# AzheeeQAQ/Game-of-life-distributed

Hardware: AMD Instinct MI355X
Metric: cell-updates/sec (GCUPS) at 1/2/4/8 MI355X; % of HBM roofline (higher is better)
Workload: dtype u32 bit-sliced (1 bit/cell)

## Files before the change

game-of-life-distributed_amd/csrc/gol_kernels.h:

```cpp
#pragma once
#include <hip/hip_runtime.h>
#include <stdint.h>

#include "gol_limits.h"
#include "gol_pad_plan.h"

namespace golk {

constexpr int kHalo = 128;
constexpr int kWave = 64;
constexpr int kTileValid = 62;
constexpr int kHalfTileValid = 30;

struct RowMap {
    int base;
    int wrap;
    int off;
    int rmax;
};

struct StepArgs {
    const uint32_t *src;
    uint32_t *dst;
    int W;
// ... 9 lines not shown

hipError_t launch_step_tb(const StepArgs &a, int depth, hipStream_t s, bool fill_skip, int wpl, bool paired = false);
int max_depth_for(int wpl);
int persist_max_depth(int wpl);
int tb_tiles(int Ww, int wpl);
hipError_t launch_step_generic(const StepArgs &a, hipStream_t s);
int tb_waves(const StepArgs &a, int wpl);
int tb_blocks_per_cu(int depth, int wpl);
int tb_wave_slots_per_cu(int depth, int wpl, bool paired);
int auto_rows_per_wave(int Ww, int rows, int depth, int wave_slots, bool fill_skip, int wpl, bool paired = false);

struct SkewArgs {
    StepArgs base;
    int tiles_x;
    int tx;
    int half;
    int nst;
    int wgt[8];
    int hcap;
    int prio_young;
    unsigned *error;
    unsigned long long *trace;
    int pairs;
};
bool skew_supported(int depth, int wpl, bool half = false, bool pr = false);
int skew_blocks_per_cu(int depth, int wpl, bool half = false, bool pr = false);
hipError_t launch_skew(const SkewArgs &p, int depth, int wpl, hipStream_t s);

struct PersistArgs {
    StepArgs base;
    uint32_t *buf0, *buf1;
    int first;
    int J;
    int half_last;
    int S;
    int S_old, S_young;
    int paired;
    int wg_tx, wg_sy;
    int cols, wg_y;
    int tiles_x;
    int nw;
    unsigned *progress;
    unsigned *error;
    long long timeout_ticks;
    unsigned long long *trace;
    int fault;
// ... 168 lines not shown
```

game-of-life-distributed_amd/csrc/gol_kernels.hip:

```cpp
#include "gol_kernels.h"
#include "gol_bits.h"
#include "gol_layout.h"
#include "gol_flip_seam.h"

#include <algorithm>
#include <climits>
#include <type_traits>
#include <utility>

namespace golk {
#ifndef GOL_LOOP_PAD
#define GOL_LOOP_PAD 0
#endif
#ifndef GOL_FILL_PHASES
#define GOL_FILL_PHASES 4
#endif

template <typename F, int... I>
__device__ __forceinline__ void static_for_impl(F &&f, std::integer_sequence<int, I...>) {
    (f(std::integral_constant<int, I>()), ...);
}
template <int N, typename F>
__device__ __forceinline__ void static_for(F &&f) {
    static_for_impl(f, std::make_integer_sequence<int, N>());
}

// ... 573 lines not shown
        if constexpr (WPL <= 2) parity_fix<1>();
        if (s < A) {
            hook(s, ii0, x0);
            stage<D, 0, WPL>(s, x0, h0, h1, cc);
        }
        if (s >= 1 && s - 1 < A) {
            hook(s - 1, ii0 + 1, x1);
            stage<D, 1, WPL>(s - 1, x1, h0, h1, cc);
        }
        if (s >= 2 && s - 2 < A) {
            hook(s - 2, ii0 + 2, x2);
            stage<D, 2, WPL>(s - 2, x2, h0, h1, cc);
        }
    }
}
#ifndef GOL_SKEW_WAIT_TRACE
#define GOL_SKEW_WAIT_TRACE 0
#endif
#ifndef GOL_SKEW_STORE_CPOL
#define GOL_SKEW_STORE_CPOL 16
#endif
template <int D>
struct SkewPlan {
    static constexpr int STEP = D > 20 ? 6 : 3;
    static constexpr int NPH = (D - 1) / STEP;
    static constexpr int P(int j) { return (j + 1) * STEP; }
    static constexpr int NROWS(int j) { return 2 * ((j + 1 < NPH ? P(j + 1) : D) - P(j)); }
    static constexpr int BASE(int j) {
        int b = 0;
        for (int i = 0; i < j; ++i) b += NROWS(i);
        return b;
    }
    static constexpr int NEXP = BASE(NPH);
    static_assert(NPH >= 1 && STEP % 3 == 0, "skew depth >= 4");
};


template <int D, int WPL>
struct PairSt {
    uint32_t a0[D][WPL], a1[D][WPL];
    uint32_t b0[D][WPL], b1[D][WPL];
    uint32_t p0[D][WPL], p1[D][WPL], p2[D][WPL];
    uint32_t c[D][WPL];
};

struct Shifted {
    uint32_t w, e;
// ... 158 lines not shown
                pair_unsum(st.p0[t][k], st.p1[t][k], st.a0[t][k], st.a1[t][k], h0[1][t][k], h1[1][t][k]);
            }
        }
}

template <int D, int LO, int WPL>
__device__ __forceinline__ void push_group_hi(Lanes<WPL> &x0, Lanes<WPL> &x1, Lanes<WPL> &x2,
                                              uint32_t (&h0)[3][D][WPL], uint32_t (&h1)[3][D][WPL],
                                              uint32_t (&cc)[3][D][WPL]) {
    parity_fix<1>();
#pragma unroll
    for (int s = LO; s < D + 2; ++s) {
        parity_fix<2>();
        if (s < D) stage<D, 0, WPL>(s, x0, h0, h1, cc);
        if (s - 1 >= LO && s - 1 < D) stage<D, 1, WPL>(s - 1, x1, h0, h1, cc);
        if (s - 2 >= LO) stage<D, 2, WPL>(s - 2, x2, h0, h1, cc);
    }
}

template <int D, int WPL, bool HALF = false, bool PR = false>
__device__ __forceinline__ uint32_t stream_skew(const StepArgs &a, int ab, int eb, int tile, bool self,
                                                uint32_t *exp_mine, const uint32_t *exp_next, int *flag_mine,
                                                int *flag_next, unsigned *error, unsigned long long *phase_tr,
                                                int dr = 0) {
    using SP = SkewPlan<D>;
    constexpr int ROW = 64 * WPL;
    constexpr int TV = HALF ? kHalfTileValid : kTileValid;
    const int lane = threadIdx.x & 63;
    const int hl = HALF ? (lane & 31) : lane;
    const int rofs = (HALF && lane >= 32) ? dr : 0;
    const int Ww = a.Ww;
    const int S = eb - ab;
    const int t0 = tile * TV * WPL;
    int col = (t0 + WPL * (hl - 1)) % Ww;
    if (col < 0) col += Ww;
    const bool keep = hl >= 1 && hl <= TV && (t0 + WPL * (hl - 1)) < Ww;
    int r = ab + rofs + a.in.off;
    const int wrap = a.in.wrap > 0 ? a.in.wrap : INT_MAX;
    if (a.in.wrap > 0) {
        r %= a.in.wrap;
        if (r < 0) r += a.in.wrap;
    }
    const uint32_t *__restrict__ src = a.src + col;
    auto load_next = [&]() -> Lanes<WPL> {
        const Lanes<WPL> v = load_row<WPL>(src + (size_t)(a.in.base + min(r, a.in.rmax)) * Ww);
        r = (r + 1 == wrap) ? 0 : r + 1;
        return v;
    };
    const __amdgpu_buffer_rsrc_t brs = __builtin_amdgcn_make_buffer_rsrc(
        a.dst + (size_t)(a.dst_base + ab + D) * Ww, (short)0, (S + (HALF ? dr : 0)) * Ww * 4, 0x00020000);
    const int clo = a.count_lo - (ab + D + rofs), chi = a.count_hi - (ab + D + rofs);
    const int colw = col + rofs * Ww;
    uint32_t cnt = 0;
    auto emit = [&](const Lanes<WPL> &y, int oi) {
        const bool ok = keep && (unsigned)oi < (unsigned)S;
// ... 47 lines not shown
            if constexpr (GOL_SKEW_WAIT_TRACE) wt0 = __builtin_amdgcn_s_memrealtime();
            x0 = vmov(n0);
            x1 = vmov(n1);
            x2 = vmov(n2);
            if constexpr (GOL_SKEW_WAIT_TRACE) {
                asm volatile("s_waitcnt vmcnt(0)" ::: "memory");
                wfill += __builtin_amdgcn_s_memrealtime() - wt0;
                ++nfill;
            }
        }
    };
    static_for<SP::NPH>([&](auto j) { fill(std::integral_constant<int, SP::P(decltype(j)::value)>()); });
    fill(std::integral_constant<int, D>());
    if (phase_tr && lane == 0) phase_tr[0] = (unsigned long long)__builtin_amdgcn_s_memrealtime();
    asm volatile("s_waitcnt lgkmcnt(0)" ::: "memory");
    if (lane == 0) __hip_atomic_store(flag_mine, 1, __ATOMIC_RELAXED, __HIP_MEMORY_SCOPE_WORKGROUP);

    Lanes<WPL> q0, q1, q2;
#pragma unroll
    for (int i = 0; i < WPL; ++i) q0.w[i] = q1.w[i] = q2.w[i] = 0u;
    int qoi = -8;
    [[maybe_unused]] PairSt<D, WPL> st;
    [[maybe_unused]] Shifted sh = {0u, 0u};
    const int kmain = S + (self ? 2 * D : 2 * SP::P(0));
    for (int i = 0; i < GOL_LOOP_PAD; ++i) asm volatile("s_nop 0");
    if constexpr (PR) {
        constexpr int KSTART = 3 * ((2 * D + 2) / 3);
        static_assert(KSTART % 6 == 0, "the pair main loop starts at an even push");
        {
            pr_enter<D, 0, WPL>(h0, h1, cc, st);
            sh = row_shifts<WPL>(x0);
            for (; k < kmain; k += 6) {
                {
                    const Lanes<WPL> n0 = load_next(), n1 = load_next(), n2 = load_next();
                    emit(q0, qoi);
                    emit(q1, qoi + 1);
                    emit(q2, qoi + 2);
                    __builtin_amdgcn_sched_barrier(0);
                    Lanes<WPL> y0 = x0, y1 = x1, y2 = x2;
                    Lanes<WPL> xn;
                    push_group_pr<D, 0, WPL>(y0, y1, y2, st, sh, n0, xn);
                    q0 = y0;
                    q1 = y1;
                    q2 = y2;
                    qoi = k - 2 * D;
                    __builtin_amdgcn_sched_barrier(0);
                    x0 = xn;
                    if constexpr (HALF) x1 = vmov(n1); else x1 = vmov_even(n1);
                    x2 = vmov(n2);
                }
                {
                    const Lanes<WPL> n0 = load_next(), n1 = load_next(), n2 = load_next();
                    emit(q0, qoi);
                    emit(q1, qoi + 1);
                    emit(q2, qoi + 2);
                    __builtin_amdgcn_sched_barrier(0);
                    Lanes<WPL> y0 = x0, y1 = x1, y2 = x2;
                    Lanes<WPL> xn;
                    push_group_pr<D, 1, WPL>(y0, y1, y2, st, sh, n0, xn);
                    q0 = y0;
                    q1 = y1;
                    q2 = y2;
                    qoi = k + 3 - 2 * D;
                    __builtin_amdgcn_sched_barrier(0);
                    x0 = xn;
                    x1 = vmov(n1);
                    x2 = vmov(n2);
                }
            }
            if constexpr (D % 3 != 0) pr_leave<D, 0, WPL>(st, h0, h1, cc);
        }
    }
    for (; !PR && k < kmain; k += 3) {
        const Lanes<WPL> n0 = load_next(), n1 = load_next(), n2 = load_next();
        emit(q0, qoi);
        emit(q1, qoi + 1);
        emit(q2, qoi + 2);
        __builtin_amdgcn_sched_barrier(0);
        Lanes<WPL> y0 = x0, y1 = x1, y2 = x2;
        push_group<D, D, WPL>(y0, y1, y2, h0, h1, cc);
        q0 = y0;
        q1 = y1;
        q2 = y2;
        qoi = k - 2 * D;
        __builtin_amdgcn_sched_barrier(0);
        if constexpr (GOL_SKEW_WAIT_TRACE) wt0 = __builtin_amdgcn_s_memrealtime();
        x0 = vmov(n0);
        x1 = vmov(n1);
        x2 = vmov(n2);
        if constexpr (GOL_SKEW_WAIT_TRACE) {
            asm volatile("s_waitcnt vmcnt(3)" ::: "memory");
            wmain += __builtin_amdgcn_s_memrealtime() - wt0;
            ++nmain;
        }
    }
    if constexpr (GOL_SKEW_WAIT_TRACE) {
        if (phase_tr && lane == 0) {
            phase_tr[32] = wmain;
            phase_tr[33] = nmain;
            phase_tr[64] = wfill;
            phase_tr[65] = nfill;
        }
    }
    if (phase_tr && lane == 0) phase_tr[1] = (unsigned long long)__builtin_amdgcn_s_memrealtime();
    if (!self) {
        if (__hip_atomic_load(flag_next, __ATOMIC_RELAXED, __HIP_MEMORY_SCOPE_WORKGROUP) == 0) {
            const long long t_start = (long long)__builtin_amdgcn_s_memrealtime();
            while (__hip_atomic_load(flag_next, __ATOMIC_RELAXED, __HIP_MEMORY_SCOPE_WORKGROUP) == 0) {
                if ((long long)__builtin_amdgcn_s_memrealtime() - t_start > 200000000ll) {
                    if (error && lane == 0) __hip_atomic_store(error, 1u, __ATOMIC_RELAXED, __HIP_MEMORY_SCOPE_SYSTEM);
                    break;
                }
                __builtin_amdgcn_s_sleep(1);
            }
        }
        asm volatile("s_waitcnt lgkmcnt(0)" ::: "memory");
// ... 101 lines not shown
    const int tile = tc * p.tx + w % p.tx, pos = w / p.tx;
    if (lane == 0) s_flag[w] = 0;
    if (threadIdx.x == 0) s_cnt = 0;
    __syncthreads();
    if (tile >= p.tiles_x) return;
    if (p.prio_young && w >= 4) __builtin_amdgcn_s_setprio(1);
    const int L = HALF ? p.base.rows_out / 2 : p.base.rows_out;
    const int A0 = (int)((int64_t)stack * L / p.nst) - D, E0 = (int)((int64_t)(stack + 1) * L / p.nst) - D;
    const int64_t Ls = (int64_t)(E0 - A0) + p.hcap;
    int cum = 0, tot = 0;
    for (int q = 0; q < sy; ++q) {
        tot += p.wgt[q];
        cum += q < pos ? p.wgt[q] : 0;
    }
    const bool bottom = pos == sy - 1;
    constexpr int G = PR ? 6 : 3;
    const int ab = A0 + (int)(Ls * cum / tot) / G * G;
    const int eb = bottom ? E0 : A0 + (int)(Ls * (cum + p.wgt[pos]) / tot) / G * G;
    const long long t_start = p.trace ? (long long)__builtin_amdgcn_s_memrealtime() : 0;
    const uint32_t cnt = stream_skew<D, WPL, HALF, PR>(p.base, ab, eb, tile, bottom, s_exp[w], bottom ? nullptr : s_exp[w + p.tx],
                                             &s_flag[w], bottom ? nullptr : &s_flag[w + p.tx], p.error,
                                             (p.trace && blockIdx.x < 1024) ? p.trace + 8 + 2 * (blockIdx.x * 64 + 16 + w)
                                                                            : nullptr,
                                             L);
    if (p.trace && lane == 0 && blockIdx.x < 1024) {
        p.trace[8 + 2 * (blockIdx.x * 64 + w)] = (unsigned long long)t_start;
        p.trace[8 + 2 * (blockIdx.x * 64 + w) + 1] = (unsigned long long)__builtin_amdgcn_s_memrealtime();
    }
    if (p.base.alive) wg_count(p.base.alive, &s_cnt, cnt, sy * min(p.tx, p.tiles_x - tc * p.tx));
}

__host__ __device__ constexpr int persist_waves(int depth, int wpl) { return depth * wpl <= 16 ? 16 : 8; }

#ifndef GOL_PERSIST_WG_COUNT
#define GOL_PERSIST_WG_COUNT 1
#endif
template <int D, int WPL, int NW>
__global__ __launch_bounds__(NW * 64) void gol_persist_kernel(PersistArgs p) {
    const int lane = threadIdx.x & 63;
    const int w = __builtin_amdgcn_readfirstlane(threadIdx.x >> 6);
    const int b = blockIdx.x;
    const int wx = b % p.cols, wy = b / p.cols;
    const int tile = wx * p.wg_tx + w % p.wg_tx;
    int r0, band, dir = 1;
    const int ry = w / p.wg_tx;
    const bool paired = p.paired != 0;
    if (paired) {
// ... 1747 lines not shown
```

game-of-life-distributed_amd/csrc/golhip_impl.h:

```cpp
#pragma once
#include <hip/hip_runtime.h>
#include <rccl/rccl.h>

#include <algorithm>
#include <atomic>
#include <chrono>
#include <condition_variable>
#include <cstdint>
#include <cstring>
#include <memory>
#include <mutex>
#include <string>
#include <vector>

#include "../../include/golhip.h"
#include "gol_kernels.h"

#define GOLHIP_HIDDEN __attribute__((visibility("hidden")))

namespace gh GOLHIP_HIDDEN {

using golk::kHalo;

int fail(int code, const char *fmt, ...) __attribute__((format(printf, 2, 3)));
// ... 68 lines not shown
    bool own_stream = false;

    uint32_t *buf[2] = {nullptr, nullptr};
    int cur = 0;
    int64_t phys_rows = 0;

    int tb_depth = 20;
    int rows_per_wave = 0;
    int cu_count = 0;
    int dev_cu = 0;
    int fill_skip = 1;
    int last_variant = 1;
    int skew = 1;
    int skew_young = 0;
    int skew_hcap = -1;
    int skew_prio = 0;
    int skew_tx = 0;
    int skew_half = 0;
    int lds_bpc[4] = {};
    int64_t lds_bpc_bytes[4] = {};
    int lds_bpc_stride[4] = {};
    int skew_bpc[gh::kNumDepths][12] = {};
    int skew_pairs = 5;
    unsigned *skew_err = nullptr;
    unsigned *skew_err_dev = nullptr;
    int lds_band = -1;
    int lds_depth = 0;
    int lds_xcd = 1;
    int lds_waves = 0;
    int lds_wg_cu = 1;
    int lds_stride = 1;
    int resident_fault = 0;
    int lds_age = 0;
    int lds_pre = 2;
    gh::DevScratch<uint32_t> lds_edge;
    int persistent = -1;
    int wpl_opt = 0;
    bool no_quads = false;
    int persist_depth = 0;
    int persist_waves = 0;
    int paired_bands = 1;
    int dummy_rows = 0;
    int persist_wg_tx = 0;
    int persist_half = 1;
    unsigned long long *d_trace = nullptr;
    unsigned *d_sync = nullptr;
// ... 188 lines not shown
```

game-of-life-distributed_amd/csrc/golhip_options.cpp:

```cpp
#include "golhip_impl.h"
#include <climits>
#include <cstdio>
#include <cstdlib>
#include <initializer_list>
#include <string>

namespace gh GOLHIP_HIDDEN {

static bool measurement_env() {
    const char *v = getenv("GOLHIP_MEASUREMENT");
    return v && !strcmp(v, "1");
}
bool test_hooks_env() {
    const char *v = getenv("GOLHIP_TEST_HOOKS");
    return v && !strcmp(v, "1");
}
bool tuning_env() {
    const char *v = getenv("GOLHIP_TUNING");
    return (v && !strcmp(v, "1")) || measurement_env();
}

namespace {

enum Consent : unsigned { kProduct = 1, kTuning = 2, kMeasurement = 4, kTestHook = 8 };

constexpr int64_t kAny = INT64_MAX;

struct Option {
    const char *key;
    unsigned consent;
    int64_t lo, hi;
    uint32_t members;
    bool or_zero;
    int golhip::*field;
    bool boolean;
    bool clears_rpw;
    int (*handler)(golhip_t h, int64_t value);
};

int set_trace(golhip_t h, int64_t value) {
    if (value && !h->d_trace) {
        if (hipMalloc(&h->d_trace, kTraceWords * sizeof(unsigned long long)) != hipSuccess)
            return fail(GOLHIP_ENOMEM, "trace buffer");
        if (hipMemsetAsync(h->d_trace, 0, kTraceWords * sizeof(unsigned long long), h->stream) != hipSuccess ||
            hipStreamSynchronize(h->stream) != hipSuccess)
            return fail(GOLHIP_EHIP, "trace buffer memset");
    }
// ... 45 lines not shown
    {"persist_depth", kTuning, RANGE(0, GOLHIP_MAX_TB_DEPTH), &golhip::persist_depth, false, false, nullptr},
    {"persist_waves", kTuning, 0, 16, bits({0, 4, 8, 16}), false, &golhip::persist_waves, false, false, nullptr},
    {"dummy_rows", kTuning, RANGE(0, kHalo), &golhip::dummy_rows, false, false, nullptr},
    {"paired_bands", kTuning, RANGE(0, 1), &golhip::paired_bands, false, true, nullptr},
    {"persist_half", kTuning, RANGE(0, 1), &golhip::persist_half, false, false, nullptr},
    {"persist_wg_tx", kTuning, RANGE(0, 16), &golhip::persist_wg_tx, false, false, nullptr},
    {"trace", kTuning, BOOLEAN, nullptr, true, false, set_trace},
    {"cu_count", kTuning, BOOLEAN, nullptr, false, true, set_cu_count},
    {"fill_skip", kTuning, BOOLEAN, &golhip::fill_skip, true, true, nullptr},
    {"skew_young", kTuning, 10, 400, 0, true, &golhip::skew_young, false, false, nullptr},
    {"skew_hcap", kTuning, RANGE(-1, 256), &golhip::skew_hcap, false, false, nullptr},
    {"skew_prio", kTuning, RANGE(0, 1), &golhip::skew_prio, false, false, nullptr},
    {"skew_half", kTuning, RANGE(-1, 1), &golhip::skew_half, false, false, nullptr},
    {"skew_tx", kTuning, RANGE(0, 2), &golhip::skew_tx, false, false, nullptr},
    {"lds_depth", kTuning, RANGE(0, 64), &golhip::lds_depth, false, false, nullptr},
    {"lds_waves", kTuning, 0, 16, bits({0, 8, 16}), false, &golhip::lds_waves, false, false, nullptr},
    {"lds_wg_cu", kTuning, RANGE(1, 2), &golhip::lds_wg_cu, false, false, nullptr},
    {"lds_age", kTuning, 25, 400, 0, true, &golhip::lds_age, false, false, nullptr},
    {"lds_pre", kTuning, RANGE(0, 64), &golhip::lds_pre, false, false, nullptr},
    {"lds_stride", kTuning, RANGE(0, 1), &golhip::lds_stride, false, false, nullptr},
    {"lds_xcd", kTuning, RANGE(0, 1), &golhip::lds_xcd, false, false, nullptr},
    {"flip_overlap", kTuning, RANGE(0, 3), &golhip::flip_overlap, false, false, nullptr},
    {"skew_pairs", kTuning, RANGE(0, 7), &golhip::skew_pairs, false, false, nullptr},
    {"halo_skip", kMeasurement, BOOLEAN, &golhip::halo_skip, true, false, nullptr},
    {"resident_fault", kTestHook, RANGE(0, 2), &golhip::resident_fault, false, false, nullptr},
    {"resident_max_turns", kTestHook, RANGE(1, golk::kResidentMaxTurns), &golhip::resident_max, false, false, nullptr},
    {"flip_debug", kMeasurement | kTestHook, RANGE(0, 7), nullptr, false, false, set_flip_debug},
};
#undef RANGE
#undef BOOLEAN

const Option *find_option(const char *key) {
    for (const Option &o : kOptions)
        if (!strcmp(key, o.key)) return &o;
    return nullptr;
}

bool accepts(const Option &o, int64_t v) {
    if (o.or_zero && v == 0) return true;
    return v >= o.lo && v <= o.hi && (!o.members || (o.members >> v & 1));
}

int refuse(const Option &o, int64_t value) {
    if (!o.members)
        return fail(GOLHIP_EINVAL, "%s %lld not in %s%lld..%lld", o.key, (long long)value, o.or_zero ? "0 or " : "",
                    (long long)o.lo, (long long)o.hi);
// ... 33 lines not shown
    return info.c_str();
}

int golhip_set_tb_depth(golhip_t h, int32_t t) {
    if (int rc = check(h)) return rc;
    if (t < 1 || t > GOLHIP_MAX_TB_DEPTH) return fail(GOLHIP_EINVAL, "tb depth %d not in 1..%d", t, GOLHIP_MAX_TB_DEPTH);
    std::lock_guard<std::mutex> g(h->mu);
    h->tb_depth = t;
    return GOLHIP_OK;
}

int golhip_set_rows_per_wave(golhip_t h, int32_t r) {
    if (int rc = check(h)) return rc;
    if (r < 0) return fail(GOLHIP_EINVAL, "rows per wave %d", r);
    std::lock_guard<std::mutex> g(h->mu);
    h->rows_per_wave = r;
    return GOLHIP_OK;
}

int golhip_set_option(golhip_t h, const char *key, int64_t value) {
    if (int rc = check(h)) return rc;
    if (!key) return fail(GOLHIP_EINVAL, "null option");
    const Option *o = find_option(key);
    if (o && (o->consent & kTuning) && !tuning_env())
        return fail(GOLHIP_EINVAL, "%s is an A/B tuning knob of the kernel plans: set GOLHIP_TUNING=1", key);
    std::lock_guard<std::mutex> g(h->mu);
    if (!o) return fail(GOLHIP_EINVAL, "unknown option %s", key);
    if (!accepts(*o, value)) return refuse(*o, value);
    if (o->handler) {
        if (int rc = o->handler(h, value)) return rc;
    } else {
        if (value && (o->consent & kMeasurement) && !measurement_env())
            return fail(GOLHIP_EINVAL, "%s gives wrong results: measurement runs only (GOLHIP_MEASUREMENT=1)", key);
        if (value && (o->consent & kTestHook) && !test_hooks_env())
            return fail(GOLHIP_EINVAL, "%s is a test hook (GOLHIP_TEST_HOOKS=1)", key);
        h->*(o->field) = o->boolean ? value != 0 : (int)value;
    }
    if (o->clears_rpw)
        for (int &c : h->auto_rpw) c = 0;
    return GOLHIP_OK;
}

}
```

game-of-life-distributed_amd/csrc/golhip_pad.cpp:

```cpp
#include "golhip_impl.h"

namespace gh GOLHIP_HIDDEN {

bool pad_applies(golhip_t h) {
    golk::PadPlan p;
    return h->W % 32 != 0 && h->torus() && !h->ringed() && golk::pad_plan(h->W, &p);
}

struct PadRule {
    int64_t min_cells, min_turns;
};
static constexpr PadRule kPadRule[] = {
    {0, 2},
    {1000 * 1000, 1},
};
static bool pad_auto(int64_t cells, int64_t nturns) {
    for (const PadRule &r : kPadRule)
        if (cells >= r.min_cells && nturns >= r.min_turns) return true;
    return false;
}

bool pad_wanted(golhip_t h, int64_t nturns) {
    if (nturns < 1 || h->pad_mode == 0 || !pad_applies(h)) return false;
    if (h->pad_mode == 1) return true;
// ... 43 lines not shown
    return GOLHIP_OK;
}

static void take_settings(golhip_t h, golhip *w) {
    w->stream = h->stream;
    w->flags = h->flags;
    if (w->wpl_opt != h->wpl_opt || w->cu_count != h->cu_count || w->fill_skip != h->fill_skip ||
        w->paired_bands != h->paired_bands)
        for (int &c : w->auto_rpw) c = 0;
    w->wpl_opt = h->wpl_opt;
    w->cu_count = h->cu_count;
    w->fill_skip = h->fill_skip;
    w->paired_bands = h->paired_bands;
    w->tb_depth = h->tb_depth;
    w->rows_per_wave = h->rows_per_wave;
    w->dummy_rows = h->dummy_rows;
    w->skew = h->skew;
    w->skew_young = h->skew_young;
    w->skew_hcap = h->skew_hcap;
    w->skew_prio = h->skew_prio;
    w->skew_tx = h->skew_tx;
    w->skew_half = h->skew_half;
    w->skew_pairs = h->skew_pairs;
    w->d_trace = h->d_trace;
}

int pad_step(golhip_t h, int64_t nturns, bool *ran) {
    *ran = false;
    if (int rc = ensure_wide(h)) {
        if (h->pad_mode == 1 || rc != GOLHIP_ENOMEM) return rc;
        h->pad_nomem = true;
        return GOLHIP_OK;
    }
    golhip *w = h->wide;
    take_settings(h, w);
    w->il = want_il(w);
    w->loaded = true;
    golk::PadArgs a{};
    golk::pad_plan(h->W, &a.plan);
    a.canon = h->cur_rows();
    a.wide = w->cur_rows();
    a.rows = h->rows;
    a.Ww = h->Ww;
    a.Wwp = w->Ww;
    w->n = Counters{};
    HIP_OR_FAIL(golk::launch_pad(a, w->il, h->stream));
// ... 169 lines not shown
```

game-of-life-distributed_amd/csrc/golhip_plan.cpp:

```cpp
#include "golhip_impl.h"
#include <climits>
#include <functional>

namespace gh GOLHIP_HIDDEN {

int largest_depth(int64_t want) {
    for (int d : kDepths)
        if (d <= want && d != 9 && d != 18) return d;
    return 1;
}
static bool special_depth(int d) { return d == 9 || d == 18; }

DepthRun depth_plan(int cap, int64_t left) {
    const int M = special_depth(cap) ? cap : largest_depth(std::max(1, cap));
    if (left <= 0) return {M, 0};
    const int64_t head = std::max<int64_t>(0, left / M - 12);
    const int t = (int)(left - head * M);
    std::vector<int> nl(t + 1, INT_MAX), mn(t + 1, 0), pick(t + 1, 0);
    nl[0] = 0;
    mn[0] = INT_MAX;
    for (int v = 1; v <= t; ++v)
        for (int d : kDepths) {
            if (d > M || d > v || nl[v - d] == INT_MAX || (special_depth(d) && M != d)) continue;
            const int n = nl[v - d] + 1, m = std::min(mn[v - d], d);
// ... 158 lines not shown
                               : golk::tb_tiles(h->Ww, wpl);
        const int Lh = half ? L / 2 : L;
        for (int tx = 1; tx <= 2; ++tx) {
            if (h->skew_tx && tx != h->skew_tx) continue;
            const int sy = 8 / tx, tcols = (tiles + tx - 1) / tx;
            const int nst = std::min(h->cu_count * bpc / tcols,
                                     Lh / (sy * (smin + hcap) - hcap));
            if (nst < 1) continue;
            if (h->skew == 1 && (int64_t)nst * tcols * 4 < (int64_t)h->cu_count * bpc * 3) continue;
            if (((double)Lh / nst + hcap + (half ? Lh : 0)) * h->Ww * 4 >= 2147483648.0) continue;
            const double per_wave = ((double)Lh / nst + hcap) / sy * (half ? 1.02 : 1.0);
            if (per_wave < best * 0.999) {
                best = per_wave;
                best_tx = tx;
                best_nst = nst;
                best_half = half;
                best_tiles = tiles;
            }
        }
    }
    if (!best_tx) return false;
    sk->tiles_x = best_tiles;
    sk->pairs = pr ? 1 : 0;
    sk->tx = best_tx;
    sk->nst = best_nst;
    sk->half = best_half;
    sk->hcap = hcap;
    return true;
}

static bool skew_fills(golhip_t h) {
    if (!h->skew || h->W % 32 != 0) return false;
    const int wpl = wpl_per_launch(h);
    int cap = std::min(h->tb_depth, golk::max_depth_for(wpl));
    if (cap == 9 && wpl != 4) cap = 8;
    const int depth = cap == 9 ? 9 : largest_depth(cap);
    golk::SkewArgs sk{};
    return skew_dims(h, depth, wpl, sched_rows(h), &sk);
}

bool skew_plan(golhip_t h, int depth, int wpl, const golk::StepArgs &a, golk::SkewArgs *sk) {
    if (!skew_dims(h, depth, wpl, a.rows_out, sk)) return false;
    if (!h->skew_err) {
        void *p = nullptr, *d = nullptr;
        if (hipHostMalloc(&p, sizeof(unsigned), hipHostMallocMapped) != hipSuccess) return false;
        if (hipHostGetDevicePointer(&d, p, 0) != hipSuccess) {
// ... 80 lines not shown
        out->pre = h->lds_pre;
        const bool whole = wpl == 2 && P2 % 64 == 0;
        out->age = h->lds_age > 0 ? h->lds_age : !whole ? 100 : waves == 16 ? 60 : 70;
    }
    return true;
}

}

using namespace gh;

extern "C" {

int golhip_halo_schedule(int32_t strip_rows, int32_t tb_depth, int32_t resident, int64_t turns_left,
                         int32_t *depth, int32_t *launches) {
    if (!depth || !launches || strip_rows <= 0 || tb_depth < 1 || tb_depth > GOLHIP_MAX_TB_DEPTH || turns_left < 1)
        return fail(GOLHIP_EINVAL, "bad halo schedule request");
    const HaloRun hr = halo_next(std::min(tb_depth, strip_rows), strip_rows, resident != 0, turns_left);
    *depth = hr.d;
    *launches = hr.k;
    return GOLHIP_OK;
}

int golhip_halo_plan(int32_t width, int32_t strip_rows, int32_t nranks, int32_t rank, int32_t depth,
                     golhip_halo_plan_t *out) {
    if (!out || width <= 0 || strip_rows <= 0 || nranks < 1 || rank < 0 || rank >= nranks || depth < 1 ||
        depth > GOLHIP_HALO_ROWS || depth > strip_rows)
        return fail(GOLHIP_EINVAL, "bad halo plan request");
    halo_plan(strip_rows, nranks, rank, depth, (width + 31) / 32, out);
    return GOLHIP_OK;
}

}
```

include/golhip.h:

```cpp
#ifndef GOLHIP_H
#define GOLHIP_H

#include <stddef.h>
#include <stdint.h>

#ifdef __cplusplus
extern "C" {
#endif

#define GOLHIP_OK 0
#define GOLHIP_EINVAL (-1)
#define GOLHIP_EHIP (-2)
#define GOLHIP_ENOMEM (-3)
#define GOLHIP_ERANGE (-4)
#define GOLHIP_ERCCL (-5)
#define GOLHIP_ECORRUPT (-6)

#define GOLHIP_FLAG_TIMING 0x1u

#define GOLHIP_UNIQUE_ID_BYTES 128
#define GOLHIP_MAX_TB_DEPTH 32
#define GOLHIP_HALO_ROWS 128

typedef struct golhip golhip;
// ... 63 lines not shown
int golhip_comm_init(golhip_t h, const uint8_t id[GOLHIP_UNIQUE_ID_BYTES], int32_t nranks, int32_t rank);
int golhip_comm_info(golhip_t h, int32_t *nranks, int32_t *rank, int32_t *ring_rows);

typedef int (*golhip_test_transport_fn)(void *user, int32_t prev_rank, int32_t next_rank, const void *send_up,
                                        const void *send_down, void *recv_top, void *recv_bottom, int64_t bytes);
int golhip_test_ring_init(golhip_t h, int32_t nranks, int32_t rank, int32_t ring_rows, golhip_test_transport_fn fn,
                          void *user);

int golhip_group_step(golhip_t *hs, int32_t n, int64_t nturns);
int golhip_group_step_ex(golhip_t *hs, int32_t n, int64_t nturns, int32_t want_flips);
int golhip_group_set_pad_step(golhip_t *hs, int32_t n, int32_t mode);

typedef struct golhip_halo_plan {
    int32_t prev_rank, next_rank;
    int32_t send_up_row, recv_top_row;
    int32_t send_down_row, recv_bottom_row;
    int32_t rows;
    int64_t bytes;
} golhip_halo_plan_t;
int golhip_halo_plan(int32_t width, int32_t strip_rows, int32_t nranks, int32_t rank, int32_t depth,
                     golhip_halo_plan_t *out);
int golhip_halo_schedule(int32_t strip_rows, int32_t tb_depth, int32_t resident, int64_t turns_left,
                         int32_t *depth, int32_t *launches);

int golhip_load_bytes(golhip_t h, const uint8_t *cells);
int golhip_load_bits(golhip_t h, const uint32_t *words);
int golhip_fill_random(golhip_t h, uint64_t seed);

int golhip_step(golhip_t h, int64_t nturns, int32_t want_flips);
int golhip_sync(golhip_t h);
int golhip_turn(golhip_t h, int64_t *turns_done);

int golhip_alive_count(golhip_t h, uint64_t *count, int64_t *at_turn);
int golhip_alive_count_global(golhip_t h, uint64_t *count, int64_t *at_turn);
int golhip_flips(golhip_t h, int32_t *xy, uint64_t cap, uint64_t *n);
int golhip_step_flips(golhip_t h, int64_t nturns, int32_t *xy, uint64_t cap, uint64_t *counts, uint64_t *n);
#define GOLHIP_FLIPS_XY 0
#define GOLHIP_FLIPS_INDEX 1
int golhip_flip_stream(golhip_t h, int64_t nturns, int32_t format, void *out, uint64_t cap, uint64_t *counts,
                       int64_t *turns_done, uint64_t *n);
int golhip_group_flip_stream(golhip_t *hs, int32_t n, int64_t nturns, int32_t format, void *out, uint64_t cap,
                             uint64_t *counts, int64_t *turns_done, uint64_t *n_entries);
int golhip_alive_cells(golhip_t h, int32_t *xy, uint64_t cap, uint64_t *n);
int golhip_snapshot_bytes(golhip_t h, uint8_t *out);
int golhip_snapshot_bits(golhip_t h, uint32_t *out);
int golhip_snapshot_rows(golhip_t h, int32_t row, int32_t nrows, uint32_t *out);
// ... 86 lines not shown
```

Baseline: 146,200.

## Add interior fast path to skew kernel main loop with linear buffer loads/stores

Computes, per band, a span of main-loop iterations whose input rows never wrap and need no alive counting. Within that span the kernel uses plain buffer loads and stores with incrementing offsets instead of the general load_next/emit paths, which handle wrapping and row mapping. This is meant to cut per-row address arithmetic and branching in the hot loop. It applies only to the paired, WPL=2, non-half, depth-18 instance, adds host-side planning helpers, and is on by default behind a tuning switch.

```diff
diff --git a/game-of-life-distributed_amd/csrc/gol_kernels.h b/game-of-life-distributed_amd/csrc/gol_kernels.h
--- a/game-of-life-distributed_amd/csrc/gol_kernels.h
+++ b/game-of-life-distributed_amd/csrc/gol_kernels.h
@@ -55,6 +55,7 @@
     unsigned *error;
     unsigned long long *trace;
     int pairs;
+    int interior;
 };
 bool skew_supported(int depth, int wpl, bool half = false, bool pr = false);
 int skew_blocks_per_cu(int depth, int wpl, bool half = false, bool pr = false);
diff --git a/game-of-life-distributed_amd/csrc/gol_kernels.hip b/game-of-life-distributed_amd/csrc/gol_kernels.hip
--- a/game-of-life-distributed_amd/csrc/gol_kernels.hip
+++ b/game-of-life-distributed_amd/csrc/gol_kernels.hip
@@ -2,6 +2,7 @@
 #include "gol_bits.h"
 #include "gol_layout.h"
 #include "gol_flip_seam.h"
+#include "gol_skew_span.h"
 
 #include <algorithm>
 #include <climits>
@@ -621,7 +622,7 @@
 #endif
 template <int D>
 struct SkewPlan {
-    static constexpr int STEP = D > 20 ? 6 : 3;
+    static constexpr int STEP = skew_phase_step(D);
     static constexpr int NPH = (D - 1) / STEP;
     static constexpr int P(int j) { return (j + 1) * STEP; }
     static constexpr int NROWS(int j) { return 2 * ((j + 1 < NPH ? P(j + 1) : D) - P(j)); }
@@ -826,7 +827,7 @@
 __device__ __forceinline__ uint32_t stream_skew(const StepArgs &a, int ab, int eb, int tile, bool self,
                                                 uint32_t *exp_mine, const uint32_t *exp_next, int *flag_mine,
                                                 int *flag_next, unsigned *error, unsigned long long *phase_tr,
-                                                int dr = 0) {
+                                                int dr = 0, bool interior = false) {
     using SP = SkewPlan<D>;
     constexpr int ROW = 64 * WPL;
     constexpr int TV = HALF ? kHalfTileValid : kTileValid;
@@ -835,6 +836,12 @@
     const int rofs = (HALF && lane >= 32) ? dr : 0;
     const int Ww = a.Ww;
     const int S = eb - ab;
+    constexpr bool SPAN = skew_interior_instance(D, WPL, HALF, PR);
+    SkewSpan span = {0, 0};
+    if constexpr (SPAN)
+        span = skew_interior_span(SkewSpanIn{ab, eb, D, self, PR, a.in.off, a.in.wrap, a.in.rmax, HALF, dr, Ww,
+                                             a.alive != nullptr && a.count_lo < a.count_hi, interior});
+    const int k_in = __builtin_amdgcn_readfirstlane(span.k_lo), k_out = __builtin_amdgcn_readfirstlane(span.k_hi);
     const int t0 = tile * TV * WPL;
     int col = (t0 + WPL * (hl - 1)) % Ww;
     if (col < 0) col += Ww;
@@ -928,20 +935,78 @@
     int qoi = -8;
     [[maybe_unused]] PairSt<D, WPL> st;
     [[maybe_unused]] Shifted sh = {0u, 0u};
-    const int kmain = S + (self ? 2 * D : 2 * SP::P(0));
+    const int kmain = skew_main_end(S, D, self);
+    const int kgen = k_in < k_out ? k_in : kmain;
+    const int ivoff = keep ? colw * 4 : INT_MAX;
+    __amdgpu_buffer_rsrc_t irs = brs;
+    int ilofs = 0;
+    int iroff = 0;
+    int isoff = 0;
+    [[maybe_unused]] auto iload = [&]() -> Lanes<WPL> {
+        Lanes<WPL> v;
+        if constexpr (WPL == 1) {
+            v.w[0] = __builtin_amdgcn_raw_buffer_load_b32(irs, ilofs, iroff, 0);
+        } else if constexpr (WPL == 2) {
+            const auto q = __builtin_amdgcn_raw_buffer_load_b64(irs, ilofs, iroff, 0);
+            v.w[0] = q[0];
+            v.w[1] = q[1];
+        } else {
+            const auto q = __builtin_amdgcn_raw_buffer_load_b128(irs, ilofs, iroff, 0);
+            v.w[0] = q[0];
+            v.w[1] = q[1];
+            v.w[2] = q[2];
+            v.w[3] = q[3];
+        }
+        iroff += Ww * 4;
+        return v;
+    };
+    [[maybe_unused]] auto istore = [&](const Lanes<WPL> &y) {
+        if constexpr (WPL == 1)
+            __builtin_amdgcn_raw_buffer_store_b32(y.w[0], brs, ivoff, isoff, GOL_SKEW_STORE_CPOL);
+        else if constexpr (WPL == 2)
+            __builtin_amdgcn_raw_buffer_store_b64((__attribute__((ext_vector_type(2))) unsigned){y.w[0], y.w[1]}, brs,
+                                                  ivoff, isoff, GOL_SKEW_STORE_CPOL);
+        else
+            __builtin_amdgcn_raw_buffer_store_b128(
+                (__attribute__((ext_vector_type(4))) unsigned){y.w[0], y.w[1], y.w[2], y.w[3]}, brs, ivoff, isoff,
+                GOL_SKEW_STORE_CPOL);
+        isoff += Ww * 4;
+    };
+    [[maybe_unused]] auto span_enter = [&]() {
+        int rb = r;
+        if constexpr (HALF) rb = min(__builtin_amdgcn_readlane(r, 0), __builtin_amdgcn_readlane(r, 32));
+        irs = __builtin_amdgcn_make_buffer_rsrc(const_cast<uint32_t *>(a.src) + (size_t)(a.in.base + rb) * Ww, (short)0,
+                                                -1, 0x00020000);
+        ilofs = (col + (r - rb) * Ww) * 4;
+        iroff = 0;
+        isoff = (k - 3 - 2 * D) * Ww * 4;
+    };
+    [[maybe_unused]] auto span_leave = [&](int rows) {
+        r += rows;
+        if (r == wrap) r = 0;
+        qoi = k - 3 - 2 * D;
+    };
     for (int i = 0; i < GOL_LOOP_PAD; ++i) asm volatile("s_nop 0");
     if constexpr (PR) {
-        constexpr int KSTART = 3 * ((2 * D + 2) / 3);
+        constexpr int KSTART = skew_main_start(D);
         static_assert(KSTART % 6 == 0, "the pair main loop starts at an even push");
         {
             pr_enter<D, 0, WPL>(h0, h1, cc, st);
             sh = row_shifts<WPL>(x0);
-            for (; k < kmain; k += 6) {
+            auto body = [&](auto in_tag) {
+                constexpr bool IN = decltype(in_tag)::value;
                 {
-                    const Lanes<WPL> n0 = load_next(), n1 = load_next(), n2 = load_next();
-                    emit(q0, qoi);
-                    emit(q1, qoi + 1);
-                    emit(q2, qoi + 2);
+                    const Lanes<WPL> n0 = IN ? iload() : load_next(), n1 = IN ? iload() : load_next(),
+                                     n2 = IN ? iload() : load_next();
+                    if constexpr (IN) {
+                        istore(q0);
+                        istore(q1);
+                        istore(q2);
+                    } else {
+                        emit(q0, qoi);
+                        emit(q1, qoi + 1);
+                        emit(q2, qoi + 2);
+                    }
                     __builtin_amdgcn_sched_barrier(0);
                     Lanes<WPL> y0 = x0, y1 = x1, y2 = x2;
                     Lanes<WPL> xn;
@@ -956,10 +1021,17 @@
                     x2 = vmov(n2);
                 }
                 {
-                    const Lanes<WPL> n0 = load_next(), n1 = load_next(), n2 = load_next();
-                    emit(q0, qoi);
-                    emit(q1, qoi + 1);
-                    emit(q2, qoi + 2);
+                    const Lanes<WPL> n0 = IN ? iload() : load_next(), n1 = IN ? iload() : load_next(),
+                                     n2 = IN ? iload() : load_next();
+                    if constexpr (IN) {
+                        istore(q0);
+                        istore(q1);
+                        istore(q2);
+                    } else {
+                        emit(q0, qoi);
+                        emit(q1, qoi + 1);
+                        emit(q2, qoi + 2);
+                    }
                     __builtin_amdgcn_sched_barrier(0);
                     Lanes<WPL> y0 = x0, y1 = x1, y2 = x2;
                     Lanes<WPL> xn;
@@ -973,31 +1045,55 @@
                     x1 = vmov(n1);
                     x2 = vmov(n2);
                 }
+            };
+            for (; k < kgen; k += 6) body(std::false_type());
+            if constexpr (SPAN) if (k_in < k_out) {
+                span_enter();
+                for (; k < k_out; k += 6) body(std::true_type());
+                span_leave(k_out - k_in);
+                for (; k < kmain; k += 6) body(std::false_type());
             }
             if constexpr (D % 3 != 0) pr_leave<D, 0, WPL>(st, h0, h1, cc);
         }
     }
-    for (; !PR && k < kmain; k += 3) {
-        const Lanes<WPL> n0 = load_next(), n1 = load_next(), n2 = load_next();
-        emit(q0, qoi);
-        emit(q1, qoi + 1);
-        emit(q2, qoi + 2);
-        __builtin_amdgcn_sched_barrier(0);
-        Lanes<WPL> y0 = x0, y1 = x1, y2 = x2;
-        push_group<D, D, WPL>(y0, y1, y2, h0, h1, cc);
-        q0 = y0;
-        q1 = y1;
-        q2 = y2;
-        qoi = k - 2 * D;
-        __builtin_amdgcn_sched_barrier(0);
-        if constexpr (GOL_SKEW_WAIT_TRACE) wt0 = __builtin_amdgcn_s_memrealtime();
-        x0 = vmov(n0);
-        x1 = vmov(n1);
-        x2 = vmov(n2);
-        if constexpr (GOL_SKEW_WAIT_TRACE) {
-            asm volatile("s_waitcnt vmcnt(3)" ::: "memory");
-            wmain += __builtin_amdgcn_s_memrealtime() - wt0;
-            ++nmain;
+    if constexpr (!PR) {
+        auto body = [&](auto in_tag) {
+            constexpr bool IN = decltype(in_tag)::value;
+            const Lanes<WPL> n0 = IN ? iload() : load_next(), n1 = IN ? iload() : load_next(),
+                             n2 = IN ? iload() : load_next();
+            if constexpr (IN) {
+                istore(q0);
+                istore(q1);
+                istore(q2);
+            } else {
+                emit(q0, qoi);
+                emit(q1, qoi + 1);
+                emit(q2, qoi + 2);
+            }
+            __builtin_amdgcn_sched_barrier(0);
+            Lanes<WPL> y0 = x0, y1 = x1, y2 = x2;
+            push_group<D, D, WPL>(y0, y1, y2, h0, h1, cc);
+            q0 = y0;
+            q1 = y1;
+            q2 = y2;
+            qoi = k - 2 * D;
+            __builtin_amdgcn_sched_barrier(0);
+            if constexpr (GOL_SKEW_WAIT_TRACE) wt0 = __builtin_amdgcn_s_memrealtime();
+            x0 = vmov(n0);
+            x1 = vmov(n1);
+            x2 = vmov(n2);
+            if constexpr (GOL_SKEW_WAIT_TRACE) {
+                asm volatile("s_waitcnt vmcnt(3)" ::: "memory");
+                wmain += __builtin_amdgcn_s_memrealtime() - wt0;
+                ++nmain;
+            }
+        };
+        for (; k < kgen; k += 3) body(std::false_type());
+        if constexpr (SPAN) if (k_in < k_out) {
+            span_enter();
+            for (; k < k_out; k += 3) body(std::true_type());
+            span_leave(k_out - k_in);
+            for (; k < kmain; k += 3) body(std::false_type());
         }
     }
     if constexpr (GOL_SKEW_WAIT_TRACE) {
@@ -1145,7 +1241,7 @@
                                              &s_flag[w], bottom ? nullptr : &s_flag[w + p.tx], p.error,
                                              (p.trace && blockIdx.x < 1024) ? p.trace + 8 + 2 * (blockIdx.x * 64 + 16 + w)
                                                                             : nullptr,
-                                             L);
+                                             L, p.interior != 0);
     if (p.trace && lane == 0 && blockIdx.x < 1024) {
         p.trace[8 + 2 * (blockIdx.x * 64 + w)] = (unsigned long long)t_start;
         p.trace[8 + 2 * (blockIdx.x * 64 + w) + 1] = (unsigned long long)__builtin_amdgcn_s_memrealtime();
diff --git a/game-of-life-distributed_amd/csrc/gol_skew_span.h b/game-of-life-distributed_amd/csrc/gol_skew_span.h
--- /dev/null
+++ b/game-of-life-distributed_amd/csrc/gol_skew_span.h
@@ -0,0 +1,141 @@
+#pragma once
+
+#if defined(__HIPCC__) || defined(__HIP__)
+#define GOL_SPAN_FN __host__ __device__ __forceinline__
+#else
+#define GOL_SPAN_FN inline
+#endif
+
+namespace golk {
+
+constexpr int skew_phase_step(int D) { return D > 20 ? 6 : 3; }
+constexpr int skew_main_start(int D) { return 3 * ((2 * D + 2) / 3); }
+constexpr int skew_main_end(int S, int D, bool self) { return S + (self ? 2 * D : 2 * skew_phase_step(D)); }
+
+struct SkewBand {
+    int ab, eb;
+    bool bottom;
+};
+GOL_SPAN_FN SkewBand skew_band(int L, int nst, int stack, int sy, int pos, const int *wgt, int hcap, int D, bool pair) {
+    const int A0 = (int)((long long)stack * L / nst) - D, E0 = (int)((long long)(stack + 1) * L / nst) - D;
+    const long long Ls = (long long)(E0 - A0) + hcap;
+    int cum = 0, tot = 0;
+    for (int q = 0; q < sy; ++q) {
+        tot += wgt[q];
+        cum += q < pos ? wgt[q] : 0;
+    }
+    const int G = pair ? 6 : 3;
+    SkewBand b;
+    b.bottom = pos == sy - 1;
+    b.ab = A0 + (int)(Ls * cum / tot) / G * G;
+    b.eb = b.bottom ? E0 : A0 + (int)(Ls * (cum + wgt[pos]) / tot) / G * G;
+    return b;
+}
+
+constexpr bool skew_interior_instance(int D, int wpl, bool half, bool pair) { return pair && wpl == 2 && !half && D == 18; }
+
+struct SkewSpan {
+    int k_lo, k_hi;
+};
+
+struct SkewSpanIn {
+    int ab, eb;
+    int D;
+    bool self;
+    bool pair;
+    int off, wrap, rmax;
+    bool half;
+    int dr;
+    int Ww;
+    bool counts;
+    bool enabled;
+};
+
+namespace span_detail {
+
+struct Rows {
+    unsigned c;
+    long long cl;
+    unsigned wrap;
+    int lim;
+};
+
+GOL_SPAN_FN long long first_row(const Rows &h, int k) {
+    return h.wrap ? (long long)((h.c + (unsigned)k) % h.wrap) : h.cl + k;
+}
+
+GOL_SPAN_FN int skip_to_good(const Rows &h, int k, int B) {
+    const long long r = first_row(h, k);
+    if (r <= h.lim) return 0;
+    if (!h.wrap || h.lim < 0) return -1;
+    return (int)(((long long)h.wrap - r + B - 1) / B) * B;
+}
+
+GOL_SPAN_FN int run_bodies(const Rows &h, int k, int B, int cap) {
+    const long long n = ((long long)h.lim - first_row(h, k)) / B + 1;
+    return n < cap ? (int)n : cap;
+}
+
+}
+
+GOL_SPAN_FN SkewSpan skew_interior_span(const SkewSpanIn &in) {
+    using namespace span_detail;
+    const int B = in.pair ? 6 : 3;
+    const int S = in.eb - in.ab, D = in.D;
+    const int k0 = skew_main_start(D);
+    SkewSpan none = {k0, k0};
+    if (!in.enabled || in.counts || S <= 0 || S > 0x7FFFFFFF - 4 * D - 64) return none;
+    if (in.half) {
+        const long long apart = in.wrap > 0 && in.wrap > in.dr ? in.wrap : in.dr;
+        if (in.dr < 0 || apart * in.Ww * 4 >= 0x7FFFFFFFll - 64) return none;
+    }
+    const int kmain = skew_main_end(S, D, in.self);
+    int lo = 2 * D + 3, hi = S + 2 * D + 4 - B;
+    if (hi > kmain) hi = kmain;
+    if (lo < k0) lo = k0;
+    const int K0 = k0 + (lo - k0 + B - 1) / B * B;
+    if (hi <= K0) return none;
+    const int K1 = K0 + (hi - K0 + B - 1) / B * B;
+    const int nh = in.half ? 2 : 1;
+    Rows h[2];
+    for (int i = 0; i < nh; ++i) {
+        const long long c = (long long)in.ab + (i ? in.dr : 0) + in.off + 3;
+        h[i].wrap = in.wrap > 0 ? (unsigned)in.wrap : 0u;
+        h[i].cl = c;
+        h[i].c = 0;
+        if (in.wrap > 0) {
+            const long long m = c % in.wrap;
+            h[i].c = (unsigned)(m < 0 ? m + in.wrap : m);
+        }
+        const long long top = in.wrap > 0 && in.wrap < (long long)in.rmax + 1 ? in.wrap : (long long)in.rmax + 1;
+        const long long lim = top - B;
+        h[i].lim = lim < -1 ? -1 : (int)lim;
+    }
+    SkewSpan best = none;
+    int k = K0;
+    for (int run = 0; run < 8 && k < K1; ++run) {
+        bool found = false;
+        for (int step = 0; step < 8 && k < K1; ++step) {
+            int skip = 0;
+            for (int i = 0; i < nh; ++i) {
+                const int s = skip_to_good(h[i], k, B);
+                if (s < 0) return best;
+                if (s > skip) skip = s;
+            }
+            if (skip == 0) {
+                found = true;
+                break;
+            }
+            if (skip >= K1 - k) return best;
+            k += skip;
+        }
+        if (!found) return best;
+        int n = (K1 - k) / B;
+        for (int i = 0; i < nh; ++i) n = run_bodies(h[i], k, B, n);
+        if (n * B > best.k_hi - best.k_lo) best = SkewSpan{k, k + n * B};
+        k += n * B;
+    }
+    return best;
+}
+
+}
diff --git a/game-of-life-distributed_amd/csrc/golhip_impl.h b/game-of-life-distributed_amd/csrc/golhip_impl.h
--- a/game-of-life-distributed_amd/csrc/golhip_impl.h
+++ b/game-of-life-distributed_amd/csrc/golhip_impl.h
@@ -114,6 +114,7 @@
     int lds_bpc_stride[4] = {};
     int skew_bpc[gh::kNumDepths][12] = {};
     int skew_pairs = 5;
+    int skew_interior = 1;
     unsigned *skew_err = nullptr;
     unsigned *skew_err_dev = nullptr;
     int lds_band = -1;
diff --git a/game-of-life-distributed_amd/csrc/golhip_options.cpp b/game-of-life-distributed_amd/csrc/golhip_options.cpp
--- a/game-of-life-distributed_amd/csrc/golhip_options.cpp
+++ b/game-of-life-distributed_amd/csrc/golhip_options.cpp
@@ -22,7 +22,7 @@
 
 namespace {
 
-enum Consent : unsigned { kProduct = 1, kTuning = 2, kMeasurement = 4, kTestHook = 8 };
+enum Consent : unsigned { kProduct = 1, kTuning = 2, kMeasurement = 4, kTestHook = 8, kPathSwitch = 16 };
 
 constexpr int64_t kAny = INT64_MAX;
 
@@ -114,6 +114,7 @@
     {"lds_xcd", kTuning, RANGE(0, 1), &golhip::lds_xcd, false, false, nullptr},
     {"flip_overlap", kTuning, RANGE(0, 3), &golhip::flip_overlap, false, false, nullptr},
     {"skew_pairs", kTuning, RANGE(0, 7), &golhip::skew_pairs, false, false, nullptr},
+    {"skew_interior", kPathSwitch, RANGE(0, 1), &golhip::skew_interior, false, false, nullptr},
     {"halo_skip", kMeasurement, BOOLEAN, &golhip::halo_skip, true, false, nullptr},
     {"resident_fault", kTestHook, RANGE(0, 2), &golhip::resident_fault, false, false, nullptr},
     {"resident_max_turns", kTestHook, RANGE(1, golk::kResidentMaxTurns), &golhip::resident_max, false, false, nullptr},
@@ -193,7 +194,7 @@
     if (int rc = check(h)) return rc;
     if (!key) return fail(GOLHIP_EINVAL, "null option");
     const Option *o = find_option(key);
-    if (o && (o->consent & kTuning) && !tuning_env())
+    if (o && (o->consent & (kTuning | kPathSwitch)) && !tuning_env())
         return fail(GOLHIP_EINVAL, "%s is an A/B tuning knob of the kernel plans: set GOLHIP_TUNING=1", key);
     std::lock_guard<std::mutex> g(h->mu);
     if (!o) return fail(GOLHIP_EINVAL, "unknown option %s", key);
diff --git a/game-of-life-distributed_amd/csrc/golhip_pad.cpp b/game-of-life-distributed_amd/csrc/golhip_pad.cpp
--- a/game-of-life-distributed_amd/csrc/golhip_pad.cpp
+++ b/game-of-life-distributed_amd/csrc/golhip_pad.cpp
@@ -89,6 +89,7 @@
     w->skew_tx = h->skew_tx;
     w->skew_half = h->skew_half;
     w->skew_pairs = h->skew_pairs;
+    w->skew_interior = h->skew_interior;
     w->d_trace = h->d_trace;
 }
 
diff --git a/game-of-life-distributed_amd/csrc/golhip_plan.cpp b/game-of-life-distributed_amd/csrc/golhip_plan.cpp
--- a/game-of-life-distributed_amd/csrc/golhip_plan.cpp
+++ b/game-of-life-distributed_amd/csrc/golhip_plan.cpp
@@ -1,4 +1,5 @@
 #include "golhip_impl.h"
+#include "gol_skew_span.h"
 #include <climits>
 #include <functional>
 
@@ -204,6 +205,7 @@
     if (!best_tx) return false;
     sk->tiles_x = best_tiles;
     sk->pairs = pr ? 1 : 0;
+    sk->interior = h->skew_interior && golk::skew_interior_instance(depth, wpl, best_half != 0, pr);
     sk->tx = best_tx;
     sk->nst = best_nst;
     sk->half = best_half;
@@ -330,6 +332,49 @@
     return GOLHIP_OK;
 }
 
+int golhip_skew_span(const golhip_skew_span_in_t *in, int32_t *k_lo, int32_t *k_hi) {
+    if (!in || !k_lo || !k_hi || in->depth < 4 || in->depth > GOLHIP_MAX_TB_DEPTH || in->eb < in->ab || in->dr < 0 || in->row_words < 1)
+        return fail(GOLHIP_EINVAL, "bad skew span request");
+    const golk::SkewSpan s = golk::skew_interior_span(golk::SkewSpanIn{
+        in->ab, in->eb, in->depth, in->self != 0, in->pair != 0, in->off, in->wrap, in->rmax, in->half != 0, in->dr, in->row_words,
+        in->counts != 0, in->enabled != 0});
+    *k_lo = s.k_lo;
+    *k_hi = s.k_hi;
+    return GOLHIP_OK;
+}
+
+int golhip_skew_interior_plan(golhip_t h, int32_t depth, int32_t ext, int32_t counts, int64_t *interior_bodies,
+                              int64_t *main_bodies) {
+    if (int rc = check(h)) return rc;
+    if (!interior_bodies || !main_bodies || depth < 1 || ext < 0) return fail(GOLHIP_EINVAL, "bad skew interior request");
+    std::lock_guard<std::mutex> g(h->mu);
+    *interior_bodies = *main_bodies = 0;
+    const bool halo = h->halo_mode();
+    if (ext > 0 && !halo) return fail(GOLHIP_EINVAL, "extended rows: strips only");
+    golk::StepArgs a = step_args(h, nullptr, halo);
+    if (ext > 0) {
+        a.rows_out = h->rows + 2 * ext;
+        a.in.off = kHalo - ext;
+        a.count_lo = ext;
+        a.count_hi = ext + h->rows;
+    }
+    golk::SkewArgs sk{};
+    const int wpl = wpl_for(h);
+    if (!skew_plan(h, depth, wpl, a, &sk)) return GOLHIP_OK;
+    const int sy = 8 / sk.tx, L = sk.half ? a.rows_out / 2 : a.rows_out, B = sk.pairs ? 6 : 3;
+    for (int stack = 0; stack < sk.nst; ++stack)
+        for (int pos = 0; pos < sy; ++pos) {
+            const golk::SkewBand b = golk::skew_band(L, sk.nst, stack, sy, pos, sk.wgt, sk.hcap, depth, sk.pairs != 0);
+            const golk::SkewSpan s = golk::skew_interior_span(golk::SkewSpanIn{
+                b.ab, b.eb, depth, b.bottom, sk.pairs != 0, a.in.off, a.in.wrap, a.in.rmax, sk.half != 0, L, a.Ww,
+                counts != 0 && a.count_lo < a.count_hi, sk.interior != 0});
+            const int k0 = golk::skew_main_start(depth), k1 = golk::skew_main_end(b.eb - b.ab, depth, b.bottom);
+            *interior_bodies += (int64_t)(s.k_hi - s.k_lo) / B * sk.tiles_x;
+            *main_bodies += (int64_t)(std::max(k1 - k0, 0) + B - 1) / B * sk.tiles_x;
+        }
+    return GOLHIP_OK;
+}
+
 int golhip_halo_plan(int32_t width, int32_t strip_rows, int32_t nranks, int32_t rank, int32_t depth,
                      golhip_halo_plan_t *out) {
     if (!out || width <= 0 || strip_rows <= 0 || nranks < 1 || rank < 0 || rank >= nranks || depth < 1 ||
diff --git a/include/golhip.h b/include/golhip.h
--- a/include/golhip.h
+++ b/include/golhip.h
@@ -109,6 +109,14 @@
                      golhip_halo_plan_t *out);
 int golhip_halo_schedule(int32_t strip_rows, int32_t tb_depth, int32_t resident, int64_t turns_left,
                          int32_t *depth, int32_t *launches);
+typedef struct golhip_skew_span_in {
+    int32_t ab, eb, depth, self, pair;
+    int32_t off, wrap, rmax;
+    int32_t half, dr, row_words, counts, enabled;
+} golhip_skew_span_in_t;
+int golhip_skew_span(const golhip_skew_span_in_t *in, int32_t *k_lo, int32_t *k_hi);
+int golhip_skew_interior_plan(golhip_t h, int32_t depth, int32_t ext, int32_t counts, int64_t *interior_bodies,
+                              int64_t *main_bodies);
 
 int golhip_load_bytes(golhip_t h, const uint8_t *cells);
 int golhip_load_bits(golhip_t h, const uint32_t *words);
```

New measurement: 149,200 (median of 6 runs). 1.02x the previous value.
